# neoncloud/mdctGAN

Hardware: AMD Instinct MI355X
Metric: train steps/sec (G+D) VCTK 12k->48k (higher is better)
Workload: dtype f32; 1 GPU; configs[1]: netG=global ngf=64 n_blocks_global=9 n_blocks_attn_g=0 num_D=2, per-GPU batch 8 x 32512 samples (128 frames x 256 bins), 12k->48k, fp32; global_batch=8, segment_length=32512, parallelism=dp1, launch=hipGraph replay

## Files before the change

mdctgan_amd/csrc/conv_co1.h:

```cpp
#pragma once

constexpr int CO1_TAPS = 64;

inline bool co1_gemm_ok(const mg_conv_geom* g) {
    const long long Mp = (long long)g->B * g->H * g->W;
    return (g->precision == MG_PRECISION_F32 || g->precision == MG_PRECISION_F16) && g->Co == 1 && g->KH * g->KW <= CO1_TAPS && g->Ci % 64 == 0 && Mp % 4 == 0 &&
           Mp * CO1_TAPS < (1LL << 29) && Mp * g->Ci < (1LL << 29);
}
inline long long co1_ldz(const mg_conv_geom* g) { return ((long long)g->B * g->H * g->W + 31) / 32 * 32; }
inline size_t co1_al(size_t b) { return (b + 255) & ~(size_t)255; }
inline size_t co1_wp_bytes(const mg_conv_geom* g) { return co1_al((size_t)CO1_TAPS * g->Ci * 4); }
inline size_t co1_zt_bytes(const mg_conv_geom* g) { return co1_al((size_t)CO1_TAPS * co1_ldz(g) * 4); }
inline int co1_wgrad_splits(const mg_conv_geom* g) {
    const int chunks = (int)(co1_ldz(g) / DG_BK), tiles = g->Ci / 64;
    int s = (256 + tiles - 1) / tiles;
    if (s > chunks / 4) s = chunks / 4;
    return s < 1 ? 1 : s;
}
inline bool co1_half(const mg_conv_geom* g) { return g->precision == MG_PRECISION_F16; }
inline size_t co1_xr_bytes(const mg_conv_geom* g) { return co1_half(g) ? co1_al((size_t)g->B * g->H * g->W * g->Ci * 4) : 0; }
inline size_t co1_fwd_ws(const mg_conv_geom* g) { return co1_wp_bytes(g) + co1_zt_bytes(g) + co1_xr_bytes(g) + 256; }
inline size_t co1_dgrad_ws(const mg_conv_geom* g) { return co1_wp_bytes(g) + co1_zt_bytes(g) + 256; }
inline size_t co1_wgrad_ws(const mg_conv_geom* g) {
    return co1_zt_bytes(g) + co1_al((size_t)co1_wgrad_splits(g) * CO1_TAPS * g->Ci * 4) + 1024 + co1_xr_bytes(g) + 256;
}

__global__ void co1_pad_w_kernel(const float* __restrict__ w, int n_real, int n_all, float* __restrict__ wp, int half) {
    for (int i = blockIdx.x * blockDim.x + threadIdx.x; i < n_all; i += gridDim.x * blockDim.x)
        wp[i] = i < n_real ? (half ? round_h(w[i]) : w[i]) : 0.0f;
}
__global__ void co1_round_kernel(const float* __restrict__ x, size_t n4, float* __restrict__ xr) {
    for (size_t i = (size_t)blockIdx.x * blockDim.x + threadIdx.x; i < n4; i += (size_t)gridDim.x * blockDim.x) {
        float4 v = ld4(x + 4 * i);
        v.x = round_h(v.x); v.y = round_h(v.y); v.z = round_h(v.z); v.w = round_h(v.w);
        *reinterpret_cast<float4*>(xr + 4 * i) = v;
    }
}

__global__ void co1_gather_kernel(Geom g, const float* __restrict__ zt, long long ldz, const float* __restrict__ bias, int act,
                                  float* __restrict__ y, int half) {
    const long long n = (long long)g.B * g.OH * g.OW;
    for (long long o = (long long)blockIdx.x * blockDim.x + threadIdx.x; o < n; o += (long long)gridDim.x * blockDim.x) {
        const int ox = (int)(o % g.OW);
        const long long r = o / g.OW;
        const int oy = (int)(r % g.OH), b = (int)(r / g.OH);
        float s = bias ? bias[0] : 0.0f;
        for (int ky = 0; ky < g.KH; ++ky) {
            int iy = oy * g.s - g.p + ky;
            if (g.reflect) iy = reflect_idx(iy, g.H);
            else if ((unsigned)iy >= (unsigned)g.H) continue;
            const float* zrow = zt + ((long long)b * g.H + iy) * g.W;
            for (int kx = 0; kx < g.KW; ++kx) {
                int ix = ox * g.s - g.p + kx;
                if (g.reflect) ix = reflect_idx(ix, g.W);
                else if ((unsigned)ix >= (unsigned)g.W) continue;
                s += zrow[(long long)(ky * g.KW + kx) * ldz + ix];
            }
        }
        s = apply_act(s, act);
        y[o] = half ? round_h(s) : s;
    }
}

__device__ __forceinline__ int co1_sources(int i, int k, int n, int on, int s, int p, int reflect, int (&out)[3]) {
    int cand[3] = {i, -i, 2 * (n - 1) - i};
    const int nc = reflect ? 3 : 1;
    int cnt = 0;
    for (int c = 0; c < nc; ++c) {
        const int u = cand[c];
        if (c == 1 && i == 0) continue;
        if (c == 2 && i == n - 1) continue;
        if (u < -p || u > n - 1 + p) continue;
        const int t = u + p - k;
        if (t < 0 || t % s != 0) continue;
        const int o = t / s;
        if (o < on) out[cnt++] = o;
    }
    return cnt;
}
template <int S>
__global__ __launch_bounds__(256) void co1_scatter_kernel(Geom g, const float* __restrict__ dy, long long ldz, float* __restrict__ gt,
                                                          int half) {
    const int tap = blockIdx.y, row = blockIdx.x * 4 + (threadIdx.x >> 6), lane = threadIdx.x & 63;
    if (row >= g.B * g.H) return;
    const int b = row / g.H, iy = row - b * g.H;
    const int ky = tap / g.KW, kx = tap - ky * g.KW;
    int oys[3];
    const int ny = co1_sources(iy, ky, g.H, g.OH, S, g.p, g.reflect, oys);
    const float* dyb = dy + (long long)b * g.OH * g.OW;
    const float* drow = dyb + (long long)(ny ? oys[0] : 0) * g.OW;
    float* out = gt + (long long)tap * ldz + (long long)row * g.W;
    for (int ix = lane; ix < g.W; ix += 64) {
        float v = 0.0f;
        if (ny) {
            const bool interior = !g.reflect || (ix > g.p && ix < g.W - 1 - g.p);
            if (ny == 1 && interior) {
                const int t = ix + g.p - kx;
                if (t >= 0 && t % S == 0 && t / S < g.OW) v = half ? round_h(drow[t / S]) : drow[t / S];
            } else {
                int oxs[3];
                const int nx = co1_sources(ix, kx, g.W, g.OW, S, g.p, g.reflect, oxs);
                for (int a = 0; a < ny; ++a)
                    for (int c = 0; c < nx; ++c) {
                        const float d = dyb[(long long)oys[a] * g.OW + oxs[c]];
                        v += half ? round_h(d) : d;
                    }
            }
        }
        out[ix] = v;
    }
}
__global__ void co1_zero_pad_kernel(float* __restrict__ gt, int taps, long long Mp, long long ldz) {
    const long long tail = ldz - Mp, n_tail = (long long)taps * tail, n_rows = (long long)(CO1_TAPS - taps) * ldz;
    for (long long i = (long long)blockIdx.x * blockDim.x + threadIdx.x; i < n_tail + n_rows; i += (long long)gridDim.x * blockDim.x) {
        if (i < n_tail) gt[(i / tail) * ldz + Mp + i % tail] = 0.0f;
        else gt[(long long)taps * ldz + (i - n_tail)] = 0.0f;
    }
}

__global__ __launch_bounds__(1024) void co1_reduce_kernel(const float* __restrict__ part, int S, long long slab, int n,
                                                          float* __restrict__ out, int accumulate) {
    __shared__ float red[16][64];
    const int i = blockIdx.x * 64 + (threadIdx.x & 63), zg = threadIdx.x >> 6;
    float s = 0.0f;
    if (i < n)
        for (int z = zg; z < S; z += 16) s += part[(long long)z * slab + i];
    red[zg][threadIdx.x & 63] = s;
    __syncthreads();
    if (zg == 0 && i < n) {
        float t = 0.0f;
#pragma unroll
        for (int q = 0; q < 16; ++q) t += red[q][threadIdx.x];
        out[i] = accumulate ? out[i] + t : t;
    }
}

__global__ void co1_sum_partial_kernel(const float* __restrict__ dy, long long n, float* __restrict__ part) {
    __shared__ float red[256];
    float s = 0.0f;
    for (long long i = (long long)blockIdx.x * blockDim.x + threadIdx.x; i < n; i += (long long)gridDim.x * blockDim.x) s += dy[i];
    red[threadIdx.x] = s;
    __syncthreads();
    for (int w = 128; w > 0; w >>= 1) {
        if ((int)threadIdx.x < w) red[threadIdx.x] += red[threadIdx.x + w];
        __syncthreads();
    }
    if (threadIdx.x == 0) part[blockIdx.x] = red[0];
}
__global__ void co1_sum_final_kernel(const float* __restrict__ part, int n, float* __restrict__ out, int accumulate) {
    __shared__ float red[256];
    red[threadIdx.x] = (int)threadIdx.x < n ? part[threadIdx.x] : 0.0f;
    __syncthreads();
    for (int w = 128; w > 0; w >>= 1) {
        if ((int)threadIdx.x < w) red[threadIdx.x] += red[threadIdx.x + w];
        __syncthreads();
    }
    if (threadIdx.x == 0) out[0] = accumulate ? out[0] + red[0] : red[0];
}

inline unsigned co1_grid(long long n) {
    long long b = (n + 255) / 256;
    return (unsigned)(b > 16384 ? 16384 : (b < 1 ? 1 : b));
}

inline void co1_gemm_z(const mg_conv_geom* g, const float* wp, const float* x, float* zt, hipStream_t st) {
    DgArgs a{};
    a.A = wp; a.B = x; a.C = zt; a.part = nullptr;
    a.M = CO1_TAPS; a.N = (int)((long long)g->B * g->H * g->W); a.K = g->Ci; a.lda = g->Ci; a.ldb = g->Ci;
    a.ldc = (int)co1_ldz(g);
    a.P = 1; a.splits = 1; a.cps = 1 << 28;
    dgemm32g_launch<64, 128, 2, 2, DG_KC, DG_KC>(a, st);
}
inline void co1_gemm_dw(const mg_conv_geom* g, const float* gt, const float* x, float* slabs, int splits, hipStream_t st) {
    DgArgs a{};
    a.A = gt; a.B = x; a.C = slabs; a.part = splits > 1 ? slabs : nullptr;
    a.M = CO1_TAPS; a.N = g->Ci; a.K = (int)co1_ldz(g); a.lda = (int)co1_ldz(g); a.ldb = g->Ci;
    a.kb = (int)((long long)g->B * g->H * g->W);
    const int chunks = a.K / DG_BK;
    a.cps = (chunks + splits - 1) / splits;
    a.splits = (chunks + a.cps - 1) / a.cps;
    a.P = 1;
    dgemm32g_launch<64, 64, 2, 2, DG_KC, DG_RC>(a, st);
}
inline void co1_gemm_dx(const mg_conv_geom* g, const float* gt, const float* wp, float* dx, hipStream_t st) {
    DgArgs a{};
    a.A = gt; a.B = wp; a.C = dx; a.part = nullptr;
    a.M = (int)((long long)g->B * g->H * g->W); a.N = g->Ci; a.K = CO1_TAPS; a.lda = (int)co1_ldz(g); a.ldb = g->Ci;
    a.P = 1; a.splits = 1; a.cps = 1 << 28;
    a.round_f16 = co1_half(g) ? 1 : 0;
    dgemm32g_launch<128, 64, 2, 2, DG_RC, DG_RC>(a, st);
}

inline void co1_pad_w(const mg_conv_geom* g, const float* w, float* wp, hipStream_t st) {
    hipLaunchKernelGGL(co1_pad_w_kernel, dim3(co1_grid(CO1_TAPS * g->Ci)), dim3(256), 0, st, w, g->KH * g->KW * g->Ci, CO1_TAPS * g->Ci, wp,
                       (int)co1_half(g));
}
inline void co1_round_x(const mg_conv_geom* g, const float* x, float* xr, hipStream_t st) {
    const size_t n4 = (size_t)g->B * g->H * g->W * g->Ci / 4;
    hipLaunchKernelGGL(co1_round_kernel, dim3(co1_grid((long long)n4)), dim3(256), 0, st, x, n4, xr);
}
int co1_fwd(const mg_conv_geom* g, const float* x, const float* w, const float* bias, float* y, int act, char* ws, hipStream_t st,
            const float* u, float* v) {
    float* wp = (float*)ws;
    float* zt = (float*)(ws + co1_wp_bytes(g));
    if (u) wp = const_cast<float*>(u);
    else co1_pad_w(g, w, wp, st);
    if (co1_half(g)) {
        float* xr = v ? v : (float*)(ws + co1_wp_bytes(g) + co1_zt_bytes(g));
        co1_round_x(g, x, xr, st);
        x = xr;
    }
    probe_begin(st);
    co1_gemm_z(g, wp, x, zt, st);
    probe_end(st);
    const Geom gg{g->B, g->H, g->W, g->Ci, g->OH, g->OW, g->Co, g->KH, g->KW, g->stride, g->pad, g->reflect};
    hipLaunchKernelGGL(co1_gather_kernel, dim3(co1_grid((long long)g->B * g->OH * g->OW)), dim3(256), 0, st, gg, (const float*)zt,
                       co1_ldz(g), bias, act, y, (int)co1_half(g));
    MG_CHECK_LAUNCH();
    return MG_OK;
}
inline void co1_scatter(const mg_conv_geom* g, const float* dy, float* gt, hipStream_t st) {
    const Geom gg{g->B, g->H, g->W, g->Ci, g->OH, g->OW, g->Co, g->KH, g->KW, g->stride, g->pad, g->reflect};
    const dim3 grid((unsigned)((g->B * g->H + 3) / 4), (unsigned)(g->KH * g->KW));
    const long long Mp = (long long)g->B * g->H * g->W, ldz = co1_ldz(g);
    const int taps = g->KH * g->KW;
    if (taps < CO1_TAPS || ldz > Mp)
        hipLaunchKernelGGL(co1_zero_pad_kernel, dim3(co1_grid((long long)taps * (ldz - Mp) + (long long)(CO1_TAPS - taps) * ldz)), dim3(256),
                           0, st, gt, taps, Mp, ldz);
    if (g->stride == 1) hipLaunchKernelGGL(co1_scatter_kernel<1>, grid, dim3(256), 0, st, gg, dy, ldz, gt, (int)co1_half(g));
    else hipLaunchKernelGGL(co1_scatter_kernel<2>, grid, dim3(256), 0, st, gg, dy, ldz, gt, (int)co1_half(g));
}
int co1_dgrad(const mg_conv_geom* g, const float* dy, const float* w, float* dx, char* ws, hipStream_t st, const float* u, float* md) {
    float* wp = (float*)ws;
    float* gt = md ? md : (float*)(ws + co1_wp_bytes(g));
    if (u) wp = const_cast<float*>(u);
    else co1_pad_w(g, w, wp, st);
    co1_scatter(g, dy, gt, st);
    probe_begin(st);
    co1_gemm_dx(g, gt, wp, dx, st);
    probe_end(st);
    MG_CHECK_LAUNCH();
    return MG_OK;
}
int co1_wgrad(const mg_conv_geom* g, const float* x, const float* dy, float* dw, float* dbias, int accumulate, char* ws,
              hipStream_t st, const float* v, const float* md) {
    float* gt = md ? const_cast<float*>(md) : (float*)ws;
    if (co1_half(g)) {
        if (v) {
            x = v;
        } else {
            float* xr = (float*)(ws + co1_zt_bytes(g) + co1_al((size_t)co1_wgrad_splits(g) * CO1_TAPS * g->Ci * 4) + 1024);
            co1_round_x(g, x, xr, st);
            x = xr;
        }
    }
    float* slabs = (float*)(ws + co1_zt_bytes(g));
    if (dbias) {
        float* part = (float*)(ws + co1_zt_bytes(g) + co1_al((size_t)co1_wgrad_splits(g) * CO1_TAPS * g->Ci * 4));
        hipLaunchKernelGGL(co1_sum_partial_kernel, dim3(256), dim3(256), 0, st, dy, (long long)g->B * g->OH * g->OW, part);
        hipLaunchKernelGGL(co1_sum_final_kernel, dim3(1), dim3(256), 0, st, (const float*)part, 256, dbias, accumulate);
    }
    const int splits = co1_wgrad_splits(g), taps = g->KH * g->KW;
    if (!md) co1_scatter(g, dy, gt, st);
    probe_begin(st);
    co1_gemm_dw(g, gt, x, slabs, splits, st);
    probe_end(st);
    const int chunks = (int)(co1_ldz(g) / DG_BK), cps = (chunks + splits - 1) / splits, real = (chunks + cps - 1) / cps;
    hipLaunchKernelGGL(co1_reduce_kernel, dim3((unsigned)((taps * g->Ci + 63) / 64)), dim3(1024), 0, st, (const float*)slabs, real,
                       (long long)CO1_TAPS * g->Ci, taps * g->Ci, dw, accumulate);
    MG_CHECK_LAUNCH();
    return MG_OK;
}
```

mdctgan_amd/csrc/conv_igemm.hip:

```cpp
#include "common.h"
#include "mdctgan_hip.h"
#include "internal.h"
#include <stdio.h>
#include <stdlib.h>
#include <cstring>
#include <type_traits>
#include <map>
#include <mutex>
#include <tuple>
#include <hip/hip_ext.h>

namespace {

constexpr int BK = 16;

struct Geom {
    int B, H, W, Ci, OH, OW, Co, KH, KW, s, p, reflect;
};

struct Batch {
    long long sa, sw, so;
    int wino_perm;
};
__device__ __forceinline__ int wino_flip(int z) {
// ... 1529 lines not shown
    const dim3 grid(wino_grid((size_t)g->Co * w.Kc / w.f.vec));
    if (w.r == R_WINO) hipLaunchKernelGGL(wino_weight_xform_kernel, grid, dim3(256), 0, st, wt, g->Co, g->Ci, U);
    else if (w.r == R_WINO4) hipLaunchKernelGGL(wino4_weight_xform_kernel, grid, dim3(256), 0, st, wt, g->Co, g->Ci, U);
    else hipLaunchKernelGGL(wino42_weight_xform_kernel, grid, dim3(256), 0, st, wt, g->Co, g->Ci, U);
}
void wino_xform_v(const WinoGeo& w, const mg_conv_geom* g, const float* x, float* V, hipStream_t st) {
    const dim3 grid(wino_grid((size_t)w.T * w.Kc / w.f.vec));
    if (w.r == R_WINO)
        hipLaunchKernelGGL(wino_input_xform_kernel, grid, dim3(256), 0, st, x, g->B, g->H, g->W, g->Ci, w.TH, w.TW, 1, g->reflect, V);
    else if (w.r == R_WINO4)
        hipLaunchKernelGGL(wino4_input_xform_kernel, grid, dim3(256), 0, st, x, g->B, g->H, g->W, g->Ci, w.TH, w.TW, V);
    else
        hipLaunchKernelGGL(wino42_input_xform_kernel, grid, dim3(256), 0, st, x, g->B, g->H, g->W, g->Ci, w.TH, w.TW, V);
}
void wino_xform_md(const WinoGeo& w, const mg_conv_geom* g, const float* dy, float* Md, hipStream_t st) {
    const dim3 grid(wino_grid((size_t)w.T * g->Co / w.f.vec));
    if (w.r == R_WINO) hipLaunchKernelGGL(wino_dy_xform_kernel, grid, dim3(256), 0, st, dy, g->B, w.TH, w.TW, g->Co, Md);
    else if (w.r == R_WINO4) hipLaunchKernelGGL(wino4_dy_xform_kernel, grid, dim3(256), 0, st, dy, g->B, w.TH, w.TW, g->Co, Md);
    else hipLaunchKernelGGL(wino42_dy_xform_kernel, grid, dim3(256), 0, st, dy, g->B, g->OH, g->OW, w.TH, w.TW, g->Co, Md);
}

int wino_fwd(const WinoGeo& w, const mg_conv_geom* g, const float* x, const float* wt, const float* bias, float* y, int act,
             float* ws, hipStream_t st, const float* u_pre, float* v_keep, bool v_filled, const WinoNorm* nrm = nullptr) {
    const WinoGemm s = wino_gemm_plan(w, 0, g);
    const WinoWs o = wino_ws(w, s, 0, g);
    float* U = u_pre ? const_cast<float*>(u_pre) : ws + o.u;
    float* V = v_keep ? v_keep : ws + o.v;
    float* Mx = ws + o.mx;
    if (!u_pre) wino_xform_u(w, g, wt, U, st);
    if (!(v_filled && v_keep)) wino_xform_v(w, g, x, V, st);
    wino_gemm(w, s, 0, g, V, U, Mx, ws + o.part, st);
    if (nrm) {
        const dim3 grid(g->Co / 32, g->B);
        const int nt = (w.TH * w.TW + 31) / 32;
#define MG_OUT_NORM(NT_) hipLaunchKernelGGL(wino_out_norm_kernel<NT_>, grid, dim3(256), 0, st, (const float*)Mx, g->B, w.TH, w.TW, g->Co, bias, *nrm, y)
#define MG_OUT_NORM_NEXT(NT_) hipLaunchKernelGGL((wino_out_norm_kernel<NT_, true>), grid, dim3(256), 0, st, (const float*)Mx, g->B, w.TH, w.TW, g->Co, bias, *nrm, y)
        if (nrm->v_next && nt == 1) MG_OUT_NORM_NEXT(1);
        else if (nrm->v_next && nt == 2) MG_OUT_NORM_NEXT(2);
        else if (nrm->v_next) return MG_ERR_ARG;
        else if (nt == 1) MG_OUT_NORM(1); else if (nt == 2) MG_OUT_NORM(2); else if (nt == 3) MG_OUT_NORM(3); else if (nt == 4) MG_OUT_NORM(4); else MG_OUT_NORM(5);
#undef MG_OUT_NORM_NEXT
#undef MG_OUT_NORM
        MG_CHECK_LAUNCH();
        return MG_OK;
    }
    const dim3 grid(wino_grid((size_t)w.T * g->Co / w.f.vec));
    if (w.r == R_WINO)
        hipLaunchKernelGGL(wino_output_xform_kernel, grid, dim3(256), 0, st, (const float*)Mx, g->B, w.TH, w.TW, g->Co, bias, act, y,
                           (int)w.hp);
    else if (w.r == R_WINO4)
        hipLaunchKernelGGL(wino4_output_xform_kernel, grid, dim3(256), 0, st, (const float*)Mx, g->B, w.TH, w.TW, g->Co, bias, act, y);
    else
        hipLaunchKernelGGL(wino42_output_xform_kernel, grid, dim3(256), 0, st, (const float*)Mx, g->B, g->OH, g->OW, w.TH, w.TW, g->Co,
                           bias, act, y);
    MG_CHECK_LAUNCH();
    return MG_OK;
}

int wino_dgrad(const WinoGeo& w, const mg_conv_geom* g, const float* dy, const float* wt, const float* bias, float* dx, int act,
               float* ws, hipStream_t st, const float* u_pre, float* md_keep, const float** addend) {
    const WinoGemm s = wino_gemm_plan(w, 1, g);
    const WinoWs o = wino_ws(w, s, 1, g);
    float* U = u_pre ? const_cast<float*>(u_pre) : ws + o.u;
    float* Md = md_keep ? md_keep : ws + o.md;
    float* dV = ws + o.dv;
    float* dd = ws + o.dd;
    if (!u_pre) wino_xform_u(w, g, wt, U, st);
    if (dy) wino_xform_md(w, g, dy, Md, st);
    wino_gemm(w, s, 1, g, Md, U, dV, ws + o.part, st);
    if (w.r == R_WINO && !w.hp && wino_dd_gather_ok(g->H, g->W, g->Ci)) {
        const int ts = w.TH * w.TW;
        const size_t lds = (size_t)ts * 16 * 8 * sizeof(float4);
        const dim3 grid(g->Ci / 32, g->B);
        const float* add = *addend;
        *addend = nullptr;
        auto go = [&](auto kern) {
            hipFuncSetAttribute((const void*)kern, hipFuncAttributeMaxDynamicSharedMemorySize, (int)lds);
            hipLaunchKernelGGL(kern, grid, dim3(256), lds, st, (const float*)dV, g->B, g->H, g->W, g->Ci, g->reflect, bias, act, dx, add);
        };
        if (ts <= 32) go(wino_dd_gather_kernel<1>); else go(wino_dd_gather_kernel<2>);
        MG_CHECK_LAUNCH();
        return MG_OK;
    }
    const dim3 grid(wino_grid((size_t)w.T * w.Kc / w.f.vec)), gx(wino_grid((size_t)g->B * g->H * g->W * g->Ci / 4));
    if (w.r == R_WINO) {
        hipLaunchKernelGGL(wino_dd_xform_kernel, grid, dim3(256), 0, st, (const float*)dV, w.T, w.Kc, dd);
        hipLaunchKernelGGL(wino_dx_gather_kernel, gx, dim3(256), 0, st, (const float*)dd, g->B, g->H, g->W, g->Ci, g->reflect, bias,
                           act, dx, (int)w.hp);
    } else {
        hipLaunchKernelGGL(wino4_dd_xform_kernel, grid, dim3(256), 0, st, (const float*)dV, w.T, w.Kc, dd);
        if (w.r == R_WINO4)
            hipLaunchKernelGGL(wino4_dx_gather_kernel, gx, dim3(256), 0, st, (const float*)dd, g->B, g->H, g->W, g->Ci, w.TH, w.TW, dx);
        else
            hipLaunchKernelGGL(wino42_dx_gather_kernel, gx, dim3(256), 0, st, (const float*)dd, g->B, g->H, g->W, g->Ci, w.TH, w.TW, dx);
    }
    MG_CHECK_LAUNCH();
    return MG_OK;
}

int wino_wgrad(const WinoGeo& w, const mg_conv_geom* g, const float* x, const float* dy, float* dw, float* dbias, int accumulate,
               float* ws, hipStream_t st, const float* v_in, const float* md_in, const mg_wino_adam* ad = nullptr) {
    const WinoGemm s = wino_gemm_plan(w, 2, g);
    const WinoWs o = wino_ws(w, s, 2, g);
    float* V = v_in ? const_cast<float*>(v_in) : ws + o.v;
    float* Md = md_in ? const_cast<float*>(md_in) : ws + o.md;
    float* dU = ws + o.du;
    if (!v_in) wino_xform_v(w, g, x, V, st);
    if (!md_in) wino_xform_md(w, g, dy, Md, st);
    wino_gemm(w, s, 2, g, Md, V, dU, ws + o.part, st);
    const dim3 grid(wino_grid((size_t)g->Co * w.Kc / w.f.vec));
    if (ad)
        hipLaunchKernelGGL(wino_adam_kernel, grid, dim3(256), 0, st, (const float*)dU, g->Co, g->Ci, dw, ad->m, ad->v, ad->u,
                           ad->state, ad->beta1, ad->beta2, ad->eps, ad->grad_scale);
    else if (w.r == R_WINO)
        hipLaunchKernelGGL(wino_dweight_xform_kernel, grid, dim3(256), 0, st, (const float*)dU, g->Co, g->Ci, dw, accumulate);
    else if (w.r == R_WINO4)
        hipLaunchKernelGGL(wino4_dweight_xform_kernel, grid, dim3(256), 0, st, (const float*)dU, g->Co, g->Ci, dw, accumulate);
    else
        hipLaunchKernelGGL(wino42_dweight_xform_kernel, grid, dim3(256), 0, st, (const float*)dU, g->Co, g->Ci, dw, accumulate);
    MG_CHECK_LAUNCH();
    if (dbias) {
        const long long M = (long long)g->B * g->OH * g->OW;
        return mg_colsum(dy, M, g->Co, dbias, accumulate, ws + o.cs, mg_colsum_workspace(M, g->Co), st);
    }
    return MG_OK;
}
bool smallc_dgrad_ok(const mg_conv_geom* g) {
    const int s = g->stride;
    return g->Ci >= 1 && g->Ci <= 4 && !g->reflect && g->Co % 4 == 0 && g->Co >= 16 &&
           (size_t)((g->KH + s - 1) / s) * ((g->KW + s - 1) / s) * g->Co * 16 <= 60 * 1024;
}
int smallc_wgrad_kind(const mg_conv_geom* g) {
    if (g->Co < 16 || ((g->stride * g->Ci) & 1)) return 0;
    if ((size_t)g->KH * (((g->OW - 1) * g->stride + g->KW) * g->Ci + 4) * sizeof(float) > 60000) return 0;
    if ((long long)g->B * g->OH > 65535LL * 32) return 0;
    if (g->KH == 4 && g->KW == 4 && g->Ci == 3) return 1;
    if (g->KH == 7 && g->KW == 7 && g->Ci == 2) return 2;
    if (g->KH == 3 && g->KW == 3 && g->Ci == 4) return 3;
    return 0;
}
struct SmallcWgradPlan { int wgs, rowlen; size_t lds; int mfma_g; };
int smallc_wgrad_mfma_groups(const mg_conv_geom* g, int rowlen) {
    if ((size_t)g->KH * rowlen > 256 * 16 || g->Co % 64 != 0) return 0;
    if (g->KH == 7 && g->KW == 7 && g->Ci == 2 && g->stride == 1) return 1;
    if (g->KH == 4 && g->KW == 4 && g->Ci == 3 && g->stride == 2) return 2;
    return 0;
}
SmallcWgradPlan smallc_wgrad_plan(const mg_conv_geom* g) {
    const int ncols = (g->OW - 1) * g->stride + g->KW;
    const int rowlen = (ncols * g->Ci + 3) / 4 * 4;
    const int mg = smallc_wgrad_mfma_groups(g, rowlen);
    return {g->B * g->OH * (mg ? mg : 1), rowlen, (size_t)g->KH * rowlen * sizeof(float), mg};
}
struct SmallcWs { size_t part, red, cs, total; };
SmallcWs smallc_wgrad_layout(const mg_conv_geom* g) {
    const SmallcWgradPlan p = smallc_wgrad_plan(g);
    const size_t n = (size_t)g->Co * g->KH * g->KW * g->Ci;
    SmallcWs w;
    w.part = 0;
    w.red = al256((size_t)p.wgs * n);
    w.cs = w.red + al256((mg_colsum_workspace(p.wgs, (int)n) + 255) / 4);
    w.total = w.cs + al256((mg_colsum_workspace((long long)g->B * g->OH * g->OW, g->Co) + 255) / 4);
    return w;
}
size_t smallc_wgrad_ws(const mg_conv_geom* g) { return smallc_wgrad_layout(g).total * sizeof(float) + 256; }
int smallc_wgrad(const mg_conv_geom* g, const float* x, const float* dy, float* dw, int accumulate, float* ws,
// ... 758 lines not shown
```

mdctgan_amd/csrc/wino4.h:

```cpp
#pragma once

namespace {

struct W4_AT { static constexpr float m[2][5] = {{1, 1, 1, 1, 0}, {0, 1, -1, 0.5f, 1}}; };
struct W4_A { static constexpr float m[5][2] = {{1, 0}, {1, 1}, {1, -1}, {1, 0.5f}, {0, 1}}; };
struct W4_G {
    static constexpr float m[5][4] = {{2, 0, 0, 0},
                                      {1, 1, 1, 1},
                                      {-1.0f / 3, 1.0f / 3, -1.0f / 3, 1.0f / 3},
                                      {-8.0f / 3, -4.0f / 3, -2.0f / 3, -1.0f / 3},
                                      {0, 0, 0, 1}};
};
struct W4_GT {
    static constexpr float m[4][5] = {{2, 1, -1.0f / 3, -8.0f / 3, 0},
                                      {0, 1, 1.0f / 3, -4.0f / 3, 0},
                                      {0, 1, -1.0f / 3, -2.0f / 3, 0},
                                      {0, 1, 1.0f / 3, -1.0f / 3, 1}};
};
struct W4_BT {
    static constexpr float m[5][5] = {{0.5f, -1, -0.5f, 1, 0},
                                      {0, -0.5f, 0.5f, 1, 0},
                                      {0, 0.5f, -1.5f, 1, 0},
                                      {0, -1, 0, 1, 0},
                                      {0, 0.5f, -1, -0.5f, 1}};
// ... 117 lines not shown
        const w4v bv = bias ? w4ld(bias + 2 * c2) : w4zero();
#pragma unroll
        for (int r = 0; r < 2; ++r)
#pragma unroll
            for (int c = 0; c < 2; ++c) {
                w4v v = make_float2(apply_act(y[r][c].x + bv.x, act), apply_act(y[r][c].y + bv.y, act));
                w4st(out + ((size_t)(b * 2 * TH + 2 * ty + r) * (2 * TW) + 2 * tx + c) * C + 2 * c2, v);
            }
    }
}

__global__ void wino4_dy_xform_kernel(const float* __restrict__ dy, int B, int TH, int TW, int C, float* __restrict__ Md) {
    const int C2 = C / 2;
    const size_t T = (size_t)B * TH * TW, total = T * C2;
    for (size_t i = (size_t)blockIdx.x * blockDim.x + threadIdx.x; i < total; i += (size_t)gridDim.x * blockDim.x) {
        const int c2 = (int)(i % C2);
        const size_t t = i / C2;
        const int tx = (int)(t % TW), ty = (int)((t / TW) % TH), b = (int)(t / ((size_t)TW * TH));
        w4v d[2][2], tmp[5][2], o[5][5];
#pragma unroll
        for (int r = 0; r < 2; ++r)
#pragma unroll
            for (int c = 0; c < 2; ++c)
                d[r][c] = w4ld(dy + ((size_t)(b * 2 * TH + 2 * ty + r) * (2 * TW) + 2 * tx + c) * C + 2 * c2);
        w4rows<W4_A, 5, 2, 2>(d, tmp);
        w4cols<W4_A, 5, 2, 5>(tmp, o);
#pragma unroll
        for (int r = 0; r < 5; ++r)
#pragma unroll
            for (int c = 0; c < 5; ++c) w4st(Md + ((size_t)(r * 5 + c) * T + t) * C + 2 * c2, o[r][c]);
    }
}

__global__ void wino4_dd_xform_kernel(const float* __restrict__ dV, long long T, int C, float* __restrict__ dd) {
    const int C2 = C / 2;
    const size_t total = (size_t)T * C2;
    for (size_t i = (size_t)blockIdx.x * blockDim.x + threadIdx.x; i < total; i += (size_t)gridDim.x * blockDim.x) {
        const int c2 = (int)(i % C2);
        const size_t t = i / C2;
        w4v v[5][5], tmp[5][5];
#pragma unroll
        for (int r = 0; r < 5; ++r)
#pragma unroll
            for (int c = 0; c < 5; ++c) v[r][c] = w4ld(dV + ((size_t)(r * 5 + c) * T + t) * C + 2 * c2);
        w4rows<W4_B, 5, 5, 5>(v, tmp);
#pragma unroll
        for (int r = 0; r < 5; ++r) {
            w4v in1[1][5], o1[1][5];
#pragma unroll
            for (int c = 0; c < 5; ++c) in1[0][c] = tmp[r][c];
            w4cols<W4_B, 5, 5, 1>(in1, o1);
#pragma unroll
            for (int c = 0; c < 5; ++c) w4st(dd + ((size_t)t * 25 + r * 5 + c) * C + 2 * c2, o1[0][c]);
        }
    }
}

__global__ void wino4_dx_gather_kernel(const float* __restrict__ dd, int B, int H, int W, int C, int TH, int TW,
                                       float* __restrict__ dx) {
    const int C4 = C / 4;
    const size_t total = (size_t)B * H * W * C4;
    for (size_t i = (size_t)blockIdx.x * blockDim.x + threadIdx.x; i < total; i += (size_t)gridDim.x * blockDim.x) {
        const int c4 = (int)(i % C4);
        const size_t p = i / C4;
        const int ix = (int)(p % W), iy = (int)((p / W) % H), b = (int)(p / ((size_t)W * H));
        float4 acc = zero4();
        const int ty_hi = (iy + 2) >> 1, tx_hi = (ix + 2) >> 1;
#pragma unroll
        for (int a = 0; a < 3; ++a) {
            const int ty = ty_hi - a, r = iy + 2 - 2 * ty;
            if (ty < 0 || ty >= TH || r > 4) continue;
#pragma unroll
            for (int e = 0; e < 3; ++e) {
                const int tx = tx_hi - e, c = ix + 2 - 2 * tx;
                if (tx < 0 || tx >= TW || c > 4) continue;
                const size_t t = ((size_t)b * TH + ty) * TW + tx;
                add4(acc, ld4(dd + (t * 25 + r * 5 + c) * C + 4 * c4));
            }
        }
        *reinterpret_cast<float4*>(dx + p * C + 4 * c4) = acc;
    }
}

__global__ void wino4_dweight_xform_kernel(const float* __restrict__ dU, int Co, int Ci, float* __restrict__ dw,
                                           int accumulate) {
    const int C2 = Ci / 2;
    const size_t total = (size_t)Co * C2;
    for (size_t i = (size_t)blockIdx.x * blockDim.x + threadIdx.x; i < total; i += (size_t)gridDim.x * blockDim.x) {
        const int c2 = (int)(i % C2), co = (int)(i / C2);
        w4v u[5][5], tmp[4][5], o[4][4];
#pragma unroll
        for (int r = 0; r < 5; ++r)
#pragma unroll
            for (int c = 0; c < 5; ++c) u[r][c] = w4ld(dU + ((size_t)(r * 5 + c) * Co + co) * Ci + 2 * c2);
        w4rows<W4_GT, 4, 5, 5>(u, tmp);
        w4cols<W4_GT, 4, 5, 4>(tmp, o);
#pragma unroll
        for (int r = 0; r < 4; ++r)
#pragma unroll
            for (int c = 0; c < 4; ++c) {
                float* q = dw + ((size_t)(co * 4 + r) * 4 + c) * Ci + 2 * c2;
                w4v v = o[r][c];
                if (accumulate) {
                    const w4v old = w4ld(q);
                    v = make_float2(old.x + v.x, old.y + v.y);
                }
                w4st(q, v);
            }
    }
}

}
```

mdctgan_amd/csrc/wino42.h:

```cpp
#pragma once

namespace {

struct W42_AT {
    static constexpr float m[4][5] = {{1, 1, 1, 1, 0}, {0, 1, -1, 0.5f, 0}, {0, 1, 1, 0.25f, 0}, {0, 1, -1, 0.125f, 1}};
};
struct W42_A {
    static constexpr float m[5][4] = {{1, 0, 0, 0}, {1, 1, 1, 1}, {1, -1, 1, -1}, {1, 0.5f, 0.25f, 0.125f}, {0, 0, 0, 1}};
};
struct W42_G {
    static constexpr float m[5][2] = {{2, 0}, {1, 1}, {-1.0f / 3, 1.0f / 3}, {-8.0f / 3, -4.0f / 3}, {0, 1}};
};
struct W42_GT {
    static constexpr float m[2][5] = {{2, 1, -1.0f / 3, -8.0f / 3, 0}, {0, 1, 1.0f / 3, -4.0f / 3, 1}};
};

struct Phase { int ay, ax, ci; };
__device__ __forceinline__ Phase w42_phase(int cp, int Ci) {
    const int a = cp / Ci;
    return {a >> 1, a & 1, cp - a * Ci};
}

__global__ void wino42_weight_xform_kernel(const float* __restrict__ w, int Co, int Ci, float* __restrict__ U) {
    const int K4 = 4 * Ci, C2 = K4 / 2;
// ... 58 lines not shown
        const int c2 = (int)(i % C2);
        const size_t t = i / C2;
        const int tx = (int)(t % TW), ty = (int)((t / TW) % TH), b = (int)(t / ((size_t)TW * TH));
        w4v m[5][5], tmp[4][5], y[4][4];
#pragma unroll
        for (int r = 0; r < 5; ++r)
#pragma unroll
            for (int c = 0; c < 5; ++c) m[r][c] = w4ld(Mx + ((size_t)(r * 5 + c) * T + t) * C + 2 * c2);
        w4rows<W42_AT, 4, 5, 5>(m, tmp);
        w4cols<W42_AT, 4, 5, 4>(tmp, y);
        const w4v bv = bias ? w4ld(bias + 2 * c2) : w4zero();
#pragma unroll
        for (int r = 0; r < 4; ++r) {
            const int oy = 4 * ty + r;
            if (oy >= OH) continue;
#pragma unroll
            for (int c = 0; c < 4; ++c) {
                const int ox = 4 * tx + c;
                if (ox >= OW) continue;
                const w4v v = make_float2(apply_act(y[r][c].x + bv.x, act), apply_act(y[r][c].y + bv.y, act));
                w4st(out + ((size_t)(b * OH + oy) * OW + ox) * C + 2 * c2, v);
            }
        }
    }
}

__global__ void wino42_dy_xform_kernel(const float* __restrict__ dy, int B, int OH, int OW, int TH, int TW, int C,
                                       float* __restrict__ Md) {
    const int C2 = C / 2;
    const size_t T = (size_t)B * TH * TW, total = T * C2;
    for (size_t i = (size_t)blockIdx.x * blockDim.x + threadIdx.x; i < total; i += (size_t)gridDim.x * blockDim.x) {
        const int c2 = (int)(i % C2);
        const size_t t = i / C2;
        const int tx = (int)(t % TW), ty = (int)((t / TW) % TH), b = (int)(t / ((size_t)TW * TH));
        w4v d[4][4], tmp[5][4];
#pragma unroll
        for (int r = 0; r < 4; ++r) {
            const int oy = 4 * ty + r;
#pragma unroll
            for (int c = 0; c < 4; ++c) {
                const int ox = 4 * tx + c;
                d[r][c] = (oy < OH && ox < OW) ? w4ld(dy + ((size_t)(b * OH + oy) * OW + ox) * C + 2 * c2) : w4zero();
            }
        }
        w4rows<W42_A, 5, 4, 4>(d, tmp);
#pragma unroll
        for (int r = 0; r < 5; ++r) {
            w4v in1[1][4], o1[1][5];
#pragma unroll
            for (int c = 0; c < 4; ++c) in1[0][c] = tmp[r][c];
            w4cols<W42_A, 5, 4, 1>(in1, o1);
#pragma unroll
            for (int c = 0; c < 5; ++c) w4st(Md + ((size_t)(r * 5 + c) * T + t) * C + 2 * c2, o1[0][c]);
        }
    }
}

__global__ void wino42_dx_gather_kernel(const float* __restrict__ dd, int B, int H, int W, int Ci, int TH, int TW,
                                        float* __restrict__ dx) {
    const int C4 = Ci / 4, K4 = 4 * Ci;
    const size_t total = (size_t)B * H * W * C4;
    for (size_t i = (size_t)blockIdx.x * blockDim.x + threadIdx.x; i < total; i += (size_t)gridDim.x * blockDim.x) {
        const int c4 = (int)(i % C4);
        const size_t p = i / C4;
        const int ix = (int)(p % W), iy = (int)((p / W) % H), b = (int)(p / ((size_t)W * H));
        const int sy = iy >> 1, sx = ix >> 1;
        const int cp = ((iy & 1) * 2 + (ix & 1)) * Ci + 4 * c4;
        float4 acc = zero4();
#pragma unroll
        for (int a = 0; a < 2; ++a) {
            const int ty = ((sy + 1) >> 2) - a, r = sy + 1 - 4 * ty;
            if (ty < 0 || ty >= TH || r > 4) continue;
#pragma unroll
            for (int e = 0; e < 2; ++e) {
                const int tx = ((sx + 1) >> 2) - e, c = sx + 1 - 4 * tx;
                if (tx < 0 || tx >= TW || c > 4) continue;
                const size_t t = ((size_t)b * TH + ty) * TW + tx;
                add4(acc, ld4(dd + (t * 25 + r * 5 + c) * K4 + cp));
            }
        }
        *reinterpret_cast<float4*>(dx + p * Ci + 4 * c4) = acc;
    }
}

__global__ void wino42_dweight_xform_kernel(const float* __restrict__ dU, int Co, int Ci, float* __restrict__ dw,
                                            int accumulate) {
    const int K4 = 4 * Ci, C2 = K4 / 2;
    const size_t total = (size_t)Co * C2;
    for (size_t i = (size_t)blockIdx.x * blockDim.x + threadIdx.x; i < total; i += (size_t)gridDim.x * blockDim.x) {
        const int cp = 2 * (int)(i % C2), co = (int)(i / C2);
        const Phase ph = w42_phase(cp, Ci);
        w4v u[5][5], tmp[2][5], o[2][2];
#pragma unroll
        for (int r = 0; r < 5; ++r)
#pragma unroll
            for (int c = 0; c < 5; ++c) u[r][c] = w4ld(dU + ((size_t)(r * 5 + c) * Co + co) * K4 + cp);
        w4rows<W42_GT, 2, 5, 5>(u, tmp);
        w4cols<W42_GT, 2, 5, 2>(tmp, o);
#pragma unroll
        for (int jy = 0; jy < 2; ++jy)
#pragma unroll
            for (int jx = 0; jx < 2; ++jx) {
                float* q = dw + ((size_t)(co * 4 + 2 * jy + ph.ay) * 4 + 2 * jx + ph.ax) * Ci + ph.ci;
                w4v v = o[jy][jx];
                if (accumulate) {
                    const w4v old = w4ld(q);
                    v = make_float2(old.x + v.x, old.y + v.y);
                }
                w4st(q, v);
            }
    }
}

}
```

Measured before the change: 91.29 steps/s.

## Fuse Winograd dgrad output transform with gather and vectorize co1 scatter

Adds a fused Winograd-4 / Winograd-4x2 dgrad kernel. It applies the inverse output transform into LDS and accumulates overlapping tile contributions in an LDS carry buffer, so the separate dd transform buffer and gather pass are no longer needed. The co1 scatter kernel now folds the zero-padding pass into itself, processes 16 rows per block, and writes float4 vectors in the interior. The co1 gather kernel gets a KW=7 specialization with an unrolled inner loop. These aim to cut global-memory round trips and launches, at the cost of heavy LDS use, which may lower occupancy, and more complex indexing.

```diff
diff --git a/mdctgan_amd/csrc/conv_co1.h b/mdctgan_amd/csrc/conv_co1.h
--- a/mdctgan_amd/csrc/conv_co1.h
+++ b/mdctgan_amd/csrc/conv_co1.h
@@ -37,6 +37,7 @@
     }
 }
 
+template <int KW_>
 __global__ void co1_gather_kernel(Geom g, const float* __restrict__ zt, long long ldz, const float* __restrict__ bias, int act,
                                   float* __restrict__ y, int half) {
     const long long n = (long long)g.B * g.OH * g.OW;
@@ -44,17 +45,19 @@
         const int ox = (int)(o % g.OW);
         const long long r = o / g.OW;
         const int oy = (int)(r % g.OH), b = (int)(r / g.OH);
+        const int KW = KW_ ? KW_ : g.KW;
         float s = bias ? bias[0] : 0.0f;
         for (int ky = 0; ky < g.KH; ++ky) {
             int iy = oy * g.s - g.p + ky;
             if (g.reflect) iy = reflect_idx(iy, g.H);
             else if ((unsigned)iy >= (unsigned)g.H) continue;
             const float* zrow = zt + ((long long)b * g.H + iy) * g.W;
-            for (int kx = 0; kx < g.KW; ++kx) {
+#pragma unroll
+            for (int kx = 0; kx < KW; ++kx) {
                 int ix = ox * g.s - g.p + kx;
                 if (g.reflect) ix = reflect_idx(ix, g.W);
                 else if ((unsigned)ix >= (unsigned)g.W) continue;
-                s += zrow[(long long)(ky * g.KW + kx) * ldz + ix];
+                s += zrow[(long long)(ky * KW + kx) * ldz + ix];
             }
         }
         s = apply_act(s, act);
@@ -78,9 +81,60 @@
     }
     return cnt;
 }
+constexpr int CO1_SCATTER_ROWS = 16;
 template <int S>
 __global__ __launch_bounds__(256) void co1_scatter_kernel(Geom g, const float* __restrict__ dy, long long ldz, float* __restrict__ gt,
-                                                          int half) {
+                                                          int half, int vec) {
+    const int tap = blockIdx.y, lane = threadIdx.x & 63;
+    const long long Mp = (long long)g.B * g.H * g.W;
+    if (blockIdx.x == 0 && (long long)threadIdx.x < ldz - Mp) gt[(long long)tap * ldz + Mp + threadIdx.x] = 0.0f;
+    const bool real = tap < g.KH * g.KW;
+    const int ky = tap / g.KW, kx = tap - ky * g.KW;
+    for (int rr = 0; rr < CO1_SCATTER_ROWS; rr += 4) {
+        const int row = blockIdx.x * CO1_SCATTER_ROWS + rr + (threadIdx.x >> 6);
+        if (row >= g.B * g.H) return;
+        const int b = row / g.H, iy = row - b * g.H;
+        int oys[3];
+        const int ny = real ? co1_sources(iy, ky, g.H, g.OH, S, g.p, g.reflect, oys) : 0;
+        const float* dyb = dy + (long long)b * g.OH * g.OW;
+        const float* drow = dyb + (long long)(ny ? oys[0] : 0) * g.OW;
+        float* out = gt + (long long)tap * ldz + (long long)row * g.W;
+        auto value = [&](int ix) {
+            float v = 0.0f;
+            if (ny) {
+                const bool interior = !g.reflect || (ix > g.p && ix < g.W - 1 - g.p);
+                if (ny == 1 && interior) {
+                    const int t = ix + g.p - kx;
+                    if (t >= 0 && t % S == 0 && t / S < g.OW) v = half ? round_h(drow[t / S]) : drow[t / S];
+                } else {
+                    int oxs[3];
+                    const int nx = co1_sources(ix, kx, g.W, g.OW, S, g.p, g.reflect, oxs);
+                    for (int a = 0; a < ny; ++a)
+                        for (int c = 0; c < nx; ++c) {
+                            const float d = dyb[(long long)oys[a] * g.OW + oxs[c]];
+                            v += half ? round_h(d) : d;
+                        }
+                }
+            }
+            return v;
+        };
+        if (vec && ny <= 1) {
+            int lo = g.reflect ? (g.p + 4) & ~3 : 0, hi = g.reflect ? (g.W - 1 - g.p) & ~3 : g.W;
+            if (hi < lo) lo = hi = 0;
+            for (int ix = lo + 4 * lane; ix < hi; ix += 256)
+                *reinterpret_cast<float4*>(out + ix) = make_float4(value(ix), value(ix + 1), value(ix + 2), value(ix + 3));
+            for (int j = lane; j < lo + g.W - hi; j += 64) {
+                const int ix = j < lo ? j : hi + (j - lo);
+                out[ix] = value(ix);
+            }
+        } else {
+            for (int ix = lane; ix < g.W; ix += 64) out[ix] = value(ix);
+        }
+    }
+}
+template <int S>
+__global__ __launch_bounds__(256) void co1_scatter_ref_kernel(Geom g, const float* __restrict__ dy, long long ldz, float* __restrict__ gt,
+                                                              int half) {
     const int tap = blockIdx.y, row = blockIdx.x * 4 + (threadIdx.x >> 6), lane = threadIdx.x & 63;
     if (row >= g.B * g.H) return;
     const int b = row / g.H, iy = row - b * g.H;
@@ -117,6 +171,7 @@
         else gt[(long long)taps * ldz + (i - n_tail)] = 0.0f;
     }
 }
+inline bool co1_vec() { return !getenv("MG_NO_CO1_VEC"); }
 
 __global__ __launch_bounds__(1024) void co1_reduce_kernel(const float* __restrict__ part, int S, long long slab, int n,
                                                           float* __restrict__ out, int accumulate) {
@@ -214,21 +269,32 @@
     co1_gemm_z(g, wp, x, zt, st);
     probe_end(st);
     const Geom gg{g->B, g->H, g->W, g->Ci, g->OH, g->OW, g->Co, g->KH, g->KW, g->stride, g->pad, g->reflect};
-    hipLaunchKernelGGL(co1_gather_kernel, dim3(co1_grid((long long)g->B * g->OH * g->OW)), dim3(256), 0, st, gg, (const float*)zt,
-                       co1_ldz(g), bias, act, y, (int)co1_half(g));
+    const dim3 grid(co1_grid((long long)g->B * g->OH * g->OW));
+    if (g->KW == 7 && co1_vec())
+        hipLaunchKernelGGL(co1_gather_kernel<7>, grid, dim3(256), 0, st, gg, (const float*)zt, co1_ldz(g), bias, act, y, (int)co1_half(g));
+    else
+        hipLaunchKernelGGL(co1_gather_kernel<0>, grid, dim3(256), 0, st, gg, (const float*)zt, co1_ldz(g), bias, act, y, (int)co1_half(g));
     MG_CHECK_LAUNCH();
     return MG_OK;
 }
 inline void co1_scatter(const mg_conv_geom* g, const float* dy, float* gt, hipStream_t st) {
     const Geom gg{g->B, g->H, g->W, g->Ci, g->OH, g->OW, g->Co, g->KH, g->KW, g->stride, g->pad, g->reflect};
-    const dim3 grid((unsigned)((g->B * g->H + 3) / 4), (unsigned)(g->KH * g->KW));
-    const long long Mp = (long long)g->B * g->H * g->W, ldz = co1_ldz(g);
-    const int taps = g->KH * g->KW;
-    if (taps < CO1_TAPS || ldz > Mp)
-        hipLaunchKernelGGL(co1_zero_pad_kernel, dim3(co1_grid((long long)taps * (ldz - Mp) + (long long)(CO1_TAPS - taps) * ldz)), dim3(256),
-                           0, st, gt, taps, Mp, ldz);
-    if (g->stride == 1) hipLaunchKernelGGL(co1_scatter_kernel<1>, grid, dim3(256), 0, st, gg, dy, ldz, gt, (int)co1_half(g));
-    else hipLaunchKernelGGL(co1_scatter_kernel<2>, grid, dim3(256), 0, st, gg, dy, ldz, gt, (int)co1_half(g));
+    const long long ldz = co1_ldz(g);
+    if (!co1_vec()) {
+        const dim3 grid((unsigned)((g->B * g->H + 3) / 4), (unsigned)(g->KH * g->KW));
+        const long long Mp = (long long)g->B * g->H * g->W;
+        const int taps = g->KH * g->KW;
+        if (taps < CO1_TAPS || ldz > Mp)
+            hipLaunchKernelGGL(co1_zero_pad_kernel, dim3(co1_grid((long long)taps * (ldz - Mp) + (long long)(CO1_TAPS - taps) * ldz)),
+                               dim3(256), 0, st, gt, taps, Mp, ldz);
+        if (g->stride == 1) hipLaunchKernelGGL(co1_scatter_ref_kernel<1>, grid, dim3(256), 0, st, gg, dy, ldz, gt, (int)co1_half(g));
+        else hipLaunchKernelGGL(co1_scatter_ref_kernel<2>, grid, dim3(256), 0, st, gg, dy, ldz, gt, (int)co1_half(g));
+        return;
+    }
+    const dim3 grid((unsigned)((g->B * g->H + CO1_SCATTER_ROWS - 1) / CO1_SCATTER_ROWS), (unsigned)CO1_TAPS);
+    const int vec = g->W % 4 == 0 && ((uintptr_t)gt & 15) == 0;
+    if (g->stride == 1) hipLaunchKernelGGL(co1_scatter_kernel<1>, grid, dim3(256), 0, st, gg, dy, ldz, gt, (int)co1_half(g), vec);
+    else hipLaunchKernelGGL(co1_scatter_kernel<2>, grid, dim3(256), 0, st, gg, dy, ldz, gt, (int)co1_half(g), vec);
 }
 int co1_dgrad(const mg_conv_geom* g, const float* dy, const float* w, float* dx, char* ws, hipStream_t st, const float* u, float* md) {
     float* wp = (float*)ws;
diff --git a/mdctgan_amd/csrc/conv_igemm.hip b/mdctgan_amd/csrc/conv_igemm.hip
--- a/mdctgan_amd/csrc/conv_igemm.hip
+++ b/mdctgan_amd/csrc/conv_igemm.hip
@@ -1635,6 +1635,24 @@
         MG_CHECK_LAUNCH();
         return MG_OK;
     }
+    if (w.r != R_WINO && !getenv("MG_NO_WINO4_DD_GATHER")) {
+        const bool f4 = w.r == R_WINO4;
+        const int SH = f4 ? g->H : (g->H + 1) / 2, SW = f4 ? g->W : (g->W + 1) / 2;
+        const int nslot = f4 ? W4Fam::NSLOT : W42Fam::NSLOT, st_rows = f4 ? W4Fam::ST : W42Fam::ST;
+        if (wino4_dd_gather_ok(w.Kc, g->Ci, w.TW, SW, nslot)) {
+            const size_t lds = wino4_dd_gather_lds(w.TW, SW, nslot);
+            const int slabs = w.Kc / W4G_CS, units = (SH + st_rows - 1) / st_rows;
+            const int upb = wino4_dd_gather_upb(slabs * g->B, units);
+            const dim3 grid(slabs, g->B, (units + upb - 1) / upb), block((w.TW * (W4G_CS / 2) + 63) / 64 * 64);
+            auto go = [&](auto kern) {
+                hipFuncSetAttribute((const void*)kern, hipFuncAttributeMaxDynamicSharedMemorySize, (int)lds);
+                hipLaunchKernelGGL(kern, grid, block, lds, st, (const float*)dV, g->B, g->H, g->W, g->Ci, w.Kc, w.TH, w.TW, upb, dx);
+            };
+            if (f4) go(wino4_dd_gather_kernel<W4Fam>); else go(wino4_dd_gather_kernel<W42Fam>);
+            MG_CHECK_LAUNCH();
+            return MG_OK;
+        }
+    }
     const dim3 grid(wino_grid((size_t)w.T * w.Kc / w.f.vec)), gx(wino_grid((size_t)g->B * g->H * g->W * g->Ci / 4));
     if (w.r == R_WINO) {
         hipLaunchKernelGGL(wino_dd_xform_kernel, grid, dim3(256), 0, st, (const float*)dV, w.T, w.Kc, dd);
diff --git a/mdctgan_amd/csrc/wino4.h b/mdctgan_amd/csrc/wino4.h
--- a/mdctgan_amd/csrc/wino4.h
+++ b/mdctgan_amd/csrc/wino4.h
@@ -223,6 +223,90 @@
     }
 }
 
+struct W4Fam {
+    static constexpr int ST = 2, OFF = 2, NA = 3, NSLOT = 4;
+    __device__ static int dom_h(int H) { return H; }
+    __device__ static int dom_w(int W) { return W; }
+    __device__ static void store(float* dx, int b, int H, int W, int Ci, int sy, int sx, int c, const float4 v) {
+        *reinterpret_cast<float4*>(dx + (((size_t)b * H + sy) * W + sx) * Ci + c) = v;
+    }
+};
+constexpr int W4G_CS = 32;
+template <class F>
+__global__ __launch_bounds__(512) void wino4_dd_gather_kernel(const float* __restrict__ dV, int B, int H, int W, int Ci, int C,
+                                                              int TH, int TW, int upb, float* __restrict__ dx) {
+    constexpr int CS = W4G_CS, TILE = 26 * CS, CP = CS / 2, CQ = CS / 4;
+    extern __shared__ __attribute__((aligned(16))) float w4g_lds[];
+    const int SH = F::dom_h(H), SW = F::dom_w(W);
+    float4* carry = reinterpret_cast<float4*>(w4g_lds + (size_t)TW * TILE);
+    const int c0 = blockIdx.x * CS, b = blockIdx.y;
+    const int s0 = blockIdx.z * upb * F::ST, s1 = min(SH, s0 + upb * F::ST);
+    const size_t T = (size_t)B * TH * TW;
+    const int t_hi = min(TH - 1, (s1 - 1 + F::OFF) / F::ST);
+    const int t_lo = s0 + F::OFF - 4 > 0 ? (s0 + F::OFF - 4 + F::ST - 1) / F::ST : 0;
+    const bool xf = (int)threadIdx.x < TW * CP;
+    const int cq = threadIdx.x % CP, txf = xf ? threadIdx.x / CP : 0;
+    w4v v[5][5];
+    auto fetch = [&](int ty) {
+        const size_t t = ((size_t)b * TH + ty) * TW + txf;
+#pragma unroll
+        for (int r = 0; r < 5; ++r)
+#pragma unroll
+            for (int c = 0; c < 5; ++c) v[r][c] = w4ld(dV + ((size_t)(r * 5 + c) * T + t) * C + c0 + 2 * cq);
+    };
+    if (xf && t_hi >= t_lo) fetch(t_hi);
+    for (int ty = t_hi; ty >= t_lo; --ty) {
+        if (xf) {
+            w4v tmp[5][5];
+            w4rows<W4_B, 5, 5, 5>(v, tmp);
+            float* pt = w4g_lds + (size_t)txf * TILE + 2 * cq;
+#pragma unroll
+            for (int r = 0; r < 5; ++r) {
+                w4v in1[1][5], o1[1][5];
+#pragma unroll
+                for (int c = 0; c < 5; ++c) in1[0][c] = tmp[r][c];
+                w4cols<W4_B, 5, 5, 1>(in1, o1);
+#pragma unroll
+                for (int c = 0; c < 5; ++c) w4st(pt + (r * 5 + c) * CS, o1[0][c]);
+            }
+            if (ty > t_lo) fetch(ty - 1);
+        }
+        __syncthreads();
+        for (int i = threadIdx.x; i < SW * CQ; i += blockDim.x) {
+            const int q = i % CQ, sx = i / CQ;
+            const int tx_hi = (sx + F::OFF) / F::ST;
+#pragma unroll
+            for (int r = 4; r >= 0; --r) {
+                const int sy = F::ST * ty - F::OFF + r;
+                if (sy < s0 || sy >= s1) continue;
+                const int first = min((sy + F::OFF) / F::ST, TH - 1);
+                const int last = sy + F::OFF - 4 > 0 ? (sy + F::OFF - 4 + F::ST - 1) / F::ST : 0;
+                float4* cs = carry + (size_t)((sy & 3) & (F::NSLOT - 1)) * SW * CQ + i;
+                float4 acc = ty == first ? zero4() : *cs;
+#pragma unroll
+                for (int e = 0; e < F::NA; ++e) {
+                    const int tx = tx_hi - e, c = sx + F::OFF - F::ST * tx;
+                    if (tx < 0 || tx >= TW || c > 4) continue;
+                    add4(acc, *reinterpret_cast<const float4*>(w4g_lds + (size_t)tx * TILE + (r * 5 + c) * CS + 4 * q));
+                }
+                if (ty == last) F::store(dx, b, H, W, Ci, sy, sx, c0 + 4 * q, acc);
+                else *cs = acc;
+            }
+        }
+        __syncthreads();
+    }
+}
+inline size_t wino4_dd_gather_lds(int TW, int SW, int nslot) {
+    return (size_t)TW * 26 * W4G_CS * sizeof(float) + (size_t)nslot * SW * (W4G_CS / 4) * sizeof(float4);
+}
+inline bool wino4_dd_gather_ok(int C, int Ci, int TW, int SW, int nslot) {
+    return C % W4G_CS == 0 && Ci % 4 == 0 && TW * (W4G_CS / 2) <= 512 && wino4_dd_gather_lds(TW, SW, nslot) <= 80 * 1024;
+}
+inline int wino4_dd_gather_upb(int slabs, int units) {
+    const int want = (1024 + slabs - 1) / slabs;
+    return (units + want - 1) / want;
+}
+
 __global__ void wino4_dweight_xform_kernel(const float* __restrict__ dU, int Co, int Ci, float* __restrict__ dw,
                                            int accumulate) {
     const int C2 = Ci / 2;
diff --git a/mdctgan_amd/csrc/wino42.h b/mdctgan_amd/csrc/wino42.h
--- a/mdctgan_amd/csrc/wino42.h
+++ b/mdctgan_amd/csrc/wino42.h
@@ -164,6 +164,17 @@
         *reinterpret_cast<float4*>(dx + p * Ci + 4 * c4) = acc;
     }
 }
+
+struct W42Fam {
+    static constexpr int ST = 4, OFF = 1, NA = 2, NSLOT = 1;
+    __device__ static int dom_h(int H) { return (H + 1) >> 1; }
+    __device__ static int dom_w(int W) { return (W + 1) >> 1; }
+    __device__ static void store(float* dx, int b, int H, int W, int Ci, int sy, int sx, int cp, const float4 v) {
+        const Phase ph = w42_phase(cp, Ci);
+        const int iy = 2 * sy + ph.ay, ix = 2 * sx + ph.ax;
+        if (iy < H && ix < W) *reinterpret_cast<float4*>(dx + (((size_t)b * H + iy) * W + ix) * Ci + ph.ci) = v;
+    }
+};
 
 __global__ void wino42_dweight_xform_kernel(const float* __restrict__ dU, int Co, int Ci, float* __restrict__ dw,
                                             int accumulate) {
```

Measured after the change: 91.53 steps/s, median of 2. About the same (+0.3%).
